# mlvlab/BLiM

Measured on AMD Instinct MI355X. Metric: candidate-pairs/sec (7B, 96+32 tok), higher is better.
Workload: dtype f16; 1 GPU; SYN v2t-VTG re-rank: Qwen2-7B dims (28 layers), seeded synthetic weights, 96 video + 32 text tokens per pair, top-16 text candidates per video query, 55 queries (880 pairs, 32560 packed tokens, 28160 label rows) per step per GPU; prefix_reuse=True, vtg_compensated=none, parallelism=query rows sharded over 1 GPU(s); RCCL all-gather of score rows at the end

## Files before the change

### blim_amd/csrc/attention.hip

```cpp
#include "attention.hpp"

#include <stdlib.h>

#include <type_traits>

#define HD 128
#define KT 32
#define QB 32

typedef __attribute__((ext_vector_type(4))) short s16x4;

template <int MAXC, bool SPLIT> struct attn_bound { static constexpr int value = MAXC <= (SPLIT ? 8 : 4) ? 512 : MAXC <= (SPLIT ? 16 : 8) ? 256 : 64; };
template <bool USE_TR, int MAXC, int DT, bool SPLIT = false, bool OUT_LO = SPLIT, bool PC = false>
__global__ __launch_bounds__((attn_bound<MAXC, SPLIT>::value)) void attn_kernel(const typename std::conditional<PC, AttnPcParams, AttnParams>::type p) {
    __shared__ __attribute__((aligned(16))) bf16_t k_lds[(SPLIT ? 2 : 1) * KT * HD];
    __shared__ __attribute__((aligned(16))) bf16_t v_lds[(SPLIT ? 2 : 1) * KT * HD];
    __shared__ uint32_t vis_lds[KT / 4];

    const int tid = threadIdx.x, nthreads = blockDim.x;
    const int lane = tid & 63;
    const int wave = tid >> 6;
    const int G = p.num_heads / p.num_kv_heads;
    const int ngrp = (int)gridDim.y / p.num_kv_heads;
    const int kh = blockIdx.y / ngrp, hg = blockIdx.y - kh * ngrp;
    const int hpg = (G + ngrp - 1) / ngrp;
    const int wave_head = hg * hpg + wave;
    const bool worker = wave < hpg && wave_head < G;
    const int head = kh * G + (worker ? wave_head : 0);
    const int blk = blockIdx.x;
    const int s = p.blk_seq[blk], q0 = p.blk_q0[blk];
    const int sstart = p.seq_start[s], slen = p.seq_len[s];
    int plen = p.pfx_len[s];
    const int pstart = plen > 0 ? p.pfx_start[s] : 0;
    const bf16_t* cbase = nullptr;
    if constexpr (PC) {
        const int slot = p.pfx_slot[s];
        if (slot >= 0 && slot < p.pc_n_slots) { cbase = p.pfx_cache + (int64_t)slot * p.pc_slot_stride; plen = min(plen, p.pc_max_len); }
    }

    const int qi = lane & 31, hf = lane >> 5;
    const int qtok = sstart + min(q0 + qi, slen - 1);
    const int qstart = p.own_start ? p.own_start[qtok] : 0;
    const int koff = p.num_heads * HD + kh * HD;
    const int voff = (p.num_heads + p.num_kv_heads) * HD + kh * HD;

    bf16x8 qf[8];
    {
        const bf16_t* qrow = p.qkv + (int64_t)qtok * p.ldq + head * HD + 8 * hf;
#pragma unroll
        for (int ks = 0; ks < 8; ++ks) qf[ks] = *(const bf16x8*)(qrow + 16 * ks);
    }
    bf16x8 qf_lo[SPLIT ? 8 : 1];
    if constexpr (SPLIT) {
        const bf16_t* qrow = p.qkv + (int64_t)qtok * p.ldq + p.v_lo_off + head * HD + 8 * hf;
#pragma unroll
        for (int ks = 0; ks < 8; ++ks) qf_lo[ks] = *(const bf16x8*)(qrow + 16 * ks);
    }

    __builtin_amdgcn_s_waitcnt(0x0F70);
    const int n_ptiles = (plen + KT - 1) / KT;
    const int own_keys = min(q0 + QB, slen);
    const int n_tiles = n_ptiles + (own_keys + KT - 1) / KT;

    f32x16 o[4];
#pragma unroll
    for (int i = 0; i < 4; ++i)
#pragma unroll
        for (int r = 0; r < 16; ++r) o[i][r] = 0.f;
    const float NEG = -1.0e30f;
    float m_run = NEG, l_run = 0.f;
    const float c_log2 = p.scale * 1.4426950408889634f;

    constexpr int NCHUNK = SPLIT ? 2048 : 1024;
    uint4 st[MAXC];
    uint8_t st_vis = 0;
#pragma unroll
    for (int i = 0; i < MAXC; ++i) st[i] = make_uint4(0, 0, 0, 0);

    auto tile_desc = [&](int t, int& base_tok, int& k0, int& seg_len, bool& causal) __attribute__((always_inline)) {
        if (t < n_ptiles) { base_tok = pstart; k0 = t * KT; seg_len = plen; causal = false; }
        else { base_tok = sstart; k0 = (t - n_ptiles) * KT; seg_len = slen; causal = true; }
    };
    auto load_tile = [&](int t) __attribute__((always_inline)) {
        int base_tok, k0, seg_len; bool causal;
        tile_desc(t, base_tok, k0, seg_len, causal);
        if constexpr (PC) {
            if (cbase != nullptr && t < n_ptiles) {
                const int ck = kh * HD, cv = p.num_kv_heads * HD + kh * HD;
#pragma unroll
                for (int i = 0; i < MAXC; ++i) {
                    const int idx = tid + i * nthreads;
                    if (idx < NCHUNK) {
                        const int isv = idx >> 9, row = (idx >> 4) & 31, ch = idx & 15;
                        const int kk = min(k0 + row, seg_len - 1);
                        st[i] = *(const uint4*)(cbase + (int64_t)kk * p.pc_ld + (isv == 0 ? ck : isv == 1 ? cv : isv == 2 ? cv + p.pc_lo_off : ck + p.pc_lo_off) + 8 * ch);
                    }
                }
                if (tid < KT) st_vis = (k0 + tid < seg_len) ? (uint8_t)1 : (uint8_t)0;
                return;
            }
        }
#pragma unroll
        for (int i = 0; i < MAXC; ++i) {
            const int idx = tid + i * nthreads;
            if (idx < NCHUNK) {
                const int isv = idx >> 9, row = (idx >> 4) & 31, ch = idx & 15;
                const int kk = min(k0 + row, seg_len - 1);
                st[i] = *(const uint4*)(p.qkv + (int64_t)(base_tok + kk) * p.ldq + (isv == 0 ? koff : isv == 1 ? voff : isv == 2 ? voff + p.v_lo_off : koff + p.v_lo_off) + 8 * ch);
            }
        }
        if (tid < KT) {
            const int kk = k0 + tid;
            st_vis = (kk < seg_len) ? p.key_visible[base_tok + kk] : (uint8_t)0;
        }
    };
    auto store_tile = [&](int t) __attribute__((always_inline)) {
        int base_tok, k0, seg_len; bool causal;
        tile_desc(t, base_tok, k0, seg_len, causal);
#pragma unroll
        for (int i = 0; i < MAXC; ++i) {
            const int idx = tid + i * nthreads;
            if (idx < NCHUNK) {
                const int isv = idx >> 9, row = (idx >> 4) & 31, ch = idx & 15;
                if (isv == 1 || isv == 2) *(uint4*)(v_lds + (isv - 1) * KT * HD + row * HD + 8 * (ch ^ ((row & 3) << 2))) = st[i];
                else *(uint4*)(k_lds + (isv >> 1) * KT * HD + row * HD + 8 * (ch ^ (row & 15))) = st[i];
            }
        }
        if (tid < KT) ((uint8_t*)vis_lds)[tid] = st_vis ? 1 : 0;
    };

    load_tile(0);
    for (int t = 0; t < n_tiles; ++t) {
#if defined(ATTN_ABLATE) && ATTN_ABLATE == 1
        if (t == 0) { __syncthreads(); store_tile(t); __syncthreads(); }
#else
        __syncthreads();
        store_tile(t);
        __syncthreads();
        if (t + 1 < n_tiles) load_tile(t + 1);
#endif
#if defined(ATTN_ABLATE) && ATTN_ABLATE == 2
        continue;
#endif
        if (!worker) continue;

        int base_tok, k0, seg_len; bool causal;
        tile_desc(t, base_tok, k0, seg_len, causal);

        f32x16 sacc;
#pragma unroll
        for (int r = 0; r < 16; ++r) sacc[r] = 0.f;
        {
            const int key = lane & 31;
#pragma unroll
            for (int ks = 0; ks < 8; ++ks) {
                const bf16x8 kf = *(const bf16x8*)(k_lds + key * HD + 8 * ((2 * ks + hf) ^ (key & 15)));
                sacc = mfma32<DT>(kf, qf[ks], sacc);
                if constexpr (SPLIT) {
                    sacc = mfma32<DT>(kf, qf_lo[ks], sacc);
                    const bf16x8 kl = *(const bf16x8*)(k_lds + KT * HD + key * HD + 8 * ((2 * ks + hf) ^ (key & 15)));
                    sacc = mfma32<DT>(kl, qf[ks], sacc);
                }
            }
        }
        float pv[16];
        const bool vis_all = (vis_lds[0] & vis_lds[1] & vis_lds[2] & vis_lds[3] & vis_lds[4] & vis_lds[5] & vis_lds[6] & vis_lds[7]) == 0x01010101u;
        if (!vis_all || (causal && (k0 + KT - 1 > q0 || p.own_start != nullptr))) {
#pragma unroll
            for (int g = 0; g < 4; ++g) {
                const uint32_t vb = vis_lds[2 * g + hf];
#pragma unroll
                for (int j = 0; j < 4; ++j) {
                    const int r = 4 * g + j;
                    const int kk = k0 + 8 * g + 4 * hf + j;
                    const bool ok = (((vb >> (8 * j)) & 0xFF) != 0) & (!causal | ((kk <= q0 + qi) & (kk >= qstart)));
                    sacc[r] = ok ? sacc[r] : NEG;
                }
            }
        }
        float tmax = NEG;
#pragma unroll
        for (int r = 0; r < 16; ++r) tmax = fmaxf(tmax, sacc[r]);
        tmax = xhalf_max(tmax);
        float m_new = m_run;
        const bool move = tmax * c_log2 > m_run * c_log2 + 8.0f;
        if (__builtin_amdgcn_ballot_w64(move) != 0) {
            m_new = move ? fmaxf(m_run, tmax) : m_run;
            const float alpha = __builtin_amdgcn_exp2f((m_run - m_new) * c_log2);
            l_run *= alpha;
#pragma unroll
            for (int i = 0; i < 4; ++i)
#pragma unroll
                for (int r = 0; r < 16; ++r) o[i][r] *= alpha;
        }
        const float mc = m_new > 0.5f * NEG ? m_new * c_log2 : 0.f;
        float rsum = 0.f;
#pragma unroll
        for (int r = 0; r < 16; ++r) {
            const float e = __builtin_amdgcn_exp2f(fmaf(sacc[r], c_log2, -mc));
            pv[r] = e;
            rsum += e;
        }
        l_run += xhalf_sum(rsum);
        m_run = m_new;

        bf16x8 pf[2], pf_lo[2];
#pragma unroll
        for (int s2 = 0; s2 < 2; ++s2) {
            uint32_t w[4], wl[4];
#pragma unroll
            for (int j = 0; j < 4; ++j) {
                const float a_ = pv[8 * s2 + 2 * j], b_ = pv[8 * s2 + 2 * j + 1];
                w[j] = pack2<DT>(a_, b_);
                if constexpr (SPLIT) wl[j] = pack2<DT>(a_ - from16<DT>(to16<DT>(a_)), b_ - from16<DT>(to16<DT>(b_)));
            }
            pf[s2] = __builtin_bit_cast(bf16x8, make_uint4(w[0], w[1], w[2], w[3]));
            if constexpr (SPLIT) pf_lo[s2] = __builtin_bit_cast(bf16x8, make_uint4(wl[0], wl[1], wl[2], wl[3]));
        }
#pragma unroll
        for (int vp = 0; vp < (SPLIT ? 2 : 1); ++vp) {
        const bf16_t* vt = v_lds + vp * KT * HD;
#pragma unroll
        for (int db = 0; db < 4; ++db) {
#pragma unroll
            for (int s2 = 0; s2 < 2; ++s2) {
                bf16x8 vf;
                if constexpr (USE_TR) {
                    const int i16 = lane & 15, g16 = (lane >> 4) & 1;
                    const int dcol = 32 * db + 16 * g16 + 4 * (i16 & 3);
                    const int ch = dcol >> 3, within = dcol & 7;
                    const int kr0 = 16 * s2 + 4 * hf + (i16 >> 2);
                    const int kr1 = kr0 + 8;
                    const s16x4 lo = __builtin_amdgcn_ds_read_tr16_b64_v4i16(
                        (__attribute__((address_space(3))) s16x4*)(vt + kr0 * HD + 8 * (ch ^ ((kr0 & 3) << 2)) + within));
                    const s16x4 hi = __builtin_amdgcn_ds_read_tr16_b64_v4i16(
                        (__attribute__((address_space(3))) s16x4*)(vt + kr1 * HD + 8 * (ch ^ ((kr1 & 3) << 2)) + within));
                    vf = (bf16x8){lo[0], lo[1], lo[2], lo[3], hi[0], hi[1], hi[2], hi[3]};
                } else {
                    const int d = 32 * db + (lane & 31);
#pragma unroll
                    for (int j = 0; j < 8; ++j) {
                        const int kr = 16 * s2 + 8 * (j >> 2) + 4 * hf + (j & 3);
                        vf[j] = (short)vt[kr * HD + 8 * ((d >> 3) ^ ((kr & 3) << 2)) + (d & 7)];
                    }
                }
                o[db] = mfma32<DT>(vf, pf[s2], o[db]);
                if constexpr (SPLIT) { if (vp == 0) o[db] = mfma32<DT>(vf, pf_lo[s2], o[db]); }
            }
        }
        }
    }

    if (!worker) return;
    if (p.out8 != nullptr) {
        const float inv = l_run > 0.f ? 1.0f / l_run : 0.f;
        float a = 0.f;
#pragma unroll
        for (int db = 0; db < 4; ++db)
#pragma unroll
            for (int r = 0; r < 16; ++r) { o[db][r] *= inv; a = fmaxf(a, fabsf(o[db][r])); }
        a = xhalf_max(a);
        int e = 0;
        if (a > 0.f) {
            int ex; const float mant = frexpf(a * (1.0f / FP8_MAX), &ex);
            e = (mant == 0.5f) ? ex - 1 : ex;
            if (ldexpf(a, -e) > FP8_MAX) e += 1;
            e = max(-127, min(127, e));
        }
        const float qs = ldexpf(1.0f, -e);
        if (q0 + qi < slen) {
            const int64_t tok = sstart + q0 + qi;
            uint8_t* orow = p.out8 + tok * p.ldo8 + head * HD;
#pragma unroll
            for (int db = 0; db < 4; ++db)
#pragma unroll
                for (int g = 0; g < 4; ++g)
                    *(uint32_t*)(orow + 32 * db + 8 * g + 4 * hf) = pack_fp8x4(o[db][4 * g] * qs, o[db][4 * g + 1] * qs, o[db][4 * g + 2] * qs, o[db][4 * g + 3] * qs);
            if (hf == 0) {
                const int rl = (int)(tok & 255);
                p.out_mx[(int64_t)head * p.mx_stride + (tok >> 8) * 256 + ((rl >> 7) * 16 + (rl & 15)) * 8 + ((rl >> 4) & 7)] = (uint8_t)(e + 127);
            }
        }
        return;
    }
    if (q0 + qi < slen) {
        const float inv = l_run > 0.f ? 1.0f / l_run : 0.f;
        bf16_t* orow = p.out + (int64_t)(sstart + q0 + qi) * p.ldo + head * HD;
        if (p.lse_out && hf == 0) p.lse_out[(int64_t)(sstart + q0 + qi) * p.num_heads + head] = l_run > 0.f ? m_run * p.scale + __logf(l_run) : 1.0e30f;
#pragma unroll
        for (int db = 0; db < 4; ++db)
#pragma unroll
            for (int g = 0; g < 4; ++g) {
                const int d = 32 * db + 8 * g + 4 * hf;
                const float x0 = o[db][4 * g] * inv, x1 = o[db][4 * g + 1] * inv, x2 = o[db][4 * g + 2] * inv, x3 = o[db][4 * g + 3] * inv;
                *(uint2*)(orow + d) = make_uint2(pack2<DT>(x0, x1), pack2<DT>(x2, x3));
                if constexpr (OUT_LO)
                    *(uint2*)(orow + p.out_lo_off + d) = make_uint2(pack2<DT>(x0 - from16<DT>(to16<DT>(x0)), x1 - from16<DT>(to16<DT>(x1))),
                                                                    pack2<DT>(x2 - from16<DT>(to16<DT>(x2)), x3 - from16<DT>(to16<DT>(x3))));
            }
    }
}

static bool stages_tile(int maxc, const dim3& block, bool split) {
    if (maxc * (int)block.x >= (split ? 2048 : 1024)) return true;
    blim_set_error("attention: %d threads x %d staging chunks do not cover a tile's %d", (int)block.x, maxc, split ? 2048 : 1024);
    return false;
}

static int launch_attention_pc(const AttnPcParams& p, int G, hipStream_t stream) {
    const dim3 grid(p.n_blocks, p.num_kv_heads), block(64 * G);
    static const int g_split = getenv("BLIM_ATTN_HEAD_GROUPS") ? atoi(getenv("BLIM_ATTN_HEAD_GROUPS")) : 2;
#define ATTN_PC(MC, SP, OL, GRID, BLOCK)                                                                                           \
    do {                                                                                                                       \
        if (!stages_tile(MC, BLOCK, SP)) return BLIM_ERR_ARG;                                                                  \
        if (p.dtype == DT_F16) hipLaunchKernelGGL((attn_kernel<true, MC, DT_F16, SP, OL, true>), GRID, BLOCK, 0, stream, p);      \
        else hipLaunchKernelGGL((attn_kernel<true, MC, DT_BF16, SP, OL, true>), GRID, BLOCK, 0, stream, p);                   \
    } while (0)
    if (p.v_lo_off != 0) {
        if (p.out_lo_off) { if (G >= 7) ATTN_PC(5, true, true, grid, block); else ATTN_PC(4, true, true, grid, dim3(512)); }
        else { if (G >= 7) ATTN_PC(5, true, false, grid, block); else ATTN_PC(4, true, false, grid, dim3(512)); }
    } else if (p.out_lo_off != 0) {
        if (G >= 7 && g_split > 1) ATTN_PC(4, false, true, dim3(p.n_blocks, p.num_kv_heads * 2), dim3(64 * ((G + 1) / 2)));
        else if (G >= 5 && g_split > 1) ATTN_PC(8, false, true, dim3(p.n_blocks, p.num_kv_heads * 2), dim3(64 * ((G + 1) / 2)));
        else if (G >= 4) ATTN_PC(4, false, true, grid, block);
        else if (G >= 2) ATTN_PC(8, false, true, grid, block);
        else ATTN_PC(16, false, true, grid, block);
    } else {
        if (G >= 7 && g_split > 1) ATTN_PC(4, false, false, dim3(p.n_blocks, p.num_kv_heads * 2), dim3(64 * ((G + 1) / 2)));
        else if (G >= 5 && g_split > 1) ATTN_PC(8, false, false, dim3(p.n_blocks, p.num_kv_heads * 2), dim3(64 * ((G + 1) / 2)));
        else if (G >= 4) ATTN_PC(4, false, false, grid, block);
        else if (G >= 2) ATTN_PC(8, false, false, grid, block);
        else ATTN_PC(16, false, false, grid, block);
    }
#undef ATTN_PC
    hipError_t e = hipGetLastError();
    if (e != hipSuccess) { blim_set_error("attention launch failed: %s", hipGetErrorString(e)); return BLIM_ERR_HIP; }
    return BLIM_OK;
}

int launch_attention_cached(const AttnPcParams& p, hipStream_t stream) {
    ARG_CHECK(p.qkv && p.out && p.key_visible && p.seq_start && p.seq_len && p.pfx_start && p.pfx_len && p.blk_seq && p.blk_q0);
    ARG_CHECK(p.n_blocks > 0 && p.num_kv_heads > 0 && p.num_heads % p.num_kv_heads == 0);
    ARG_CHECK(p.ldq % 8 == 0 && p.ldo % 4 == 0);
    ARG_CHECK(p.pfx_cache && p.pfx_slot && p.pc_n_slots > 0 && p.pc_max_len > 0 && p.pc_ld % 8 == 0 && p.pc_lo_off % 8 == 0 && p.pc_slot_stride % 8 == 0 && p.pc_lo_off >= 0);
    ARG_CHECK((p.dtype == DT_F16 || p.dtype == DT_BF16) && p.v_lo_off >= 0 && p.out_lo_off >= 0 && p.v_lo_off % 8 == 0 && p.out_lo_off % 4 == 0);
    if (p.out8 || p.lse_out) { blim_set_error("attention: the prefix-cache forms write a 16-bit output and no lse"); return BLIM_ERR_ARG; }
    if (p.v_lo_off != 0 && p.pc_lo_off == 0) { blim_set_error("attention: a compensated call needs a prefix cache that holds lo parts"); return BLIM_ERR_ARG; }
    const int G = p.num_heads / p.num_kv_heads;
    if (G > 8) { blim_set_error("attention: %d query heads per kv head > 8 unsupported", G); return BLIM_ERR_ARG; }
    return launch_attention_pc(p, G, stream);
}

int launch_attention(const AttnParams& p, int use_tr_read, hipStream_t stream) {
    ARG_CHECK(p.qkv && p.out && p.key_visible && p.seq_start && p.seq_len && p.pfx_start && p.pfx_len && p.blk_seq && p.blk_q0);
    ARG_CHECK(p.n_blocks > 0 && p.num_kv_heads > 0 && p.num_heads % p.num_kv_heads == 0);
    ARG_CHECK(p.ldq % 8 == 0 && p.ldo % 4 == 0);
    const int G = p.num_heads / p.num_kv_heads;
    if (G > 8) { blim_set_error("attention: %d query heads per kv head > 8 unsupported", G); return BLIM_ERR_ARG; }
    const dim3 grid(p.n_blocks, p.num_kv_heads), block(64 * G);
    if (p.v_lo_off != 0 || p.out_lo_off != 0)
        ARG_CHECK((p.dtype == DT_F16 || p.dtype == DT_BF16) && p.v_lo_off >= 0 && p.out_lo_off >= 0 && p.v_lo_off % 8 == 0 && p.out_lo_off % 4 == 0 && !p.out8);
    if (p.v_lo_off != 0) {
#define ATTN_SPLIT(MC, BLOCK)                                                                                                       \
        do {                                                                                                                      \
            if (!stages_tile(MC, BLOCK, true)) return BLIM_ERR_ARG;                                                               \
            if (p.out_lo_off) {                                                                                                   \
                if (p.dtype == DT_F16) hipLaunchKernelGGL((attn_kernel<true, MC, DT_F16, true>), grid, BLOCK, 0, stream, p);       \
                else hipLaunchKernelGGL((attn_kernel<true, MC, DT_BF16, true>), grid, BLOCK, 0, stream, p);                    \
            } else {                                                                                                              \
                if (p.dtype == DT_F16) hipLaunchKernelGGL((attn_kernel<true, MC, DT_F16, true, false>), grid, BLOCK, 0, stream, p); \
                else hipLaunchKernelGGL((attn_kernel<true, MC, DT_BF16, true, false>), grid, BLOCK, 0, stream, p);              \
            }                                                                                                                     \
        } while (0)
        if (G >= 7) ATTN_SPLIT(5, block);
        else ATTN_SPLIT(4, dim3(512));
#undef ATTN_SPLIT
        hipError_t e2 = hipGetLastError();
        if (e2 != hipSuccess) { blim_set_error("attention launch failed: %s", hipGetErrorString(e2)); return BLIM_ERR_HIP; }
        return BLIM_OK;
    }
    static const int g_split = getenv("BLIM_ATTN_HEAD_GROUPS") ? atoi(getenv("BLIM_ATTN_HEAD_GROUPS")) : 2;
    if (p.out_lo_off != 0) {
#define ATTN_LO(MC, GRID, BLOCK)                                                                                                   \
        do {                                                                                                                     \
            if (!stages_tile(MC, BLOCK, false)) return BLIM_ERR_ARG;                                                             \
            if (p.dtype == DT_F16) hipLaunchKernelGGL((attn_kernel<true, MC, DT_F16, false, true>), GRID, BLOCK, 0, stream, p);   \
            else hipLaunchKernelGGL((attn_kernel<true, MC, DT_BF16, false, true>), GRID, BLOCK, 0, stream, p);                \
        } while (0)
        if (G >= 7 && g_split > 1) ATTN_LO(4, dim3(p.n_blocks, p.num_kv_heads * 2), dim3(64 * ((G + 1) / 2)));
        else if (G >= 5 && g_split > 1) ATTN_LO(8, dim3(p.n_blocks, p.num_kv_heads * 2), dim3(64 * ((G + 1) / 2)));
        else if (G >= 4) ATTN_LO(4, grid, block);
        else if (G >= 2) ATTN_LO(8, grid, block);
        else ATTN_LO(16, grid, block);
#undef ATTN_LO
        hipError_t e3 = hipGetLastError();
        if (e3 != hipSuccess) { blim_set_error("attention launch failed: %s", hipGetErrorString(e3)); return BLIM_ERR_HIP; }
        return BLIM_OK;
    }
#define ATTN_LAUNCH(TR, MC)                                                                             \
    do {                                                                                            \
        if (!stages_tile(MC, block, false)) return BLIM_ERR_ARG;                                    \
        if (p.dtype == DT_F16) hipLaunchKernelGGL((attn_kernel<TR, MC, DT_F16>), grid, block, 0, stream, p); \
        else hipLaunchKernelGGL((attn_kernel<TR, MC, DT_BF16>), grid, block, 0, stream, p);                \
    } while (0)
    if (G >= 5 && g_split > 1 && use_tr_read && !p.out8) {
        const int hpg = (G + 1) / 2;
        const dim3 grid2(p.n_blocks, p.num_kv_heads * 2), block2(64 * hpg);
        if (!stages_tile(hpg >= 4 ? 4 : 8, block2, false)) return BLIM_ERR_ARG;
        if (hpg >= 4) {
            if (p.dtype == DT_F16) hipLaunchKernelGGL((attn_kernel<true, 4, DT_F16>), grid2, block2, 0, stream, p);
            else hipLaunchKernelGGL((attn_kernel<true, 4, DT_BF16>), grid2, block2, 0, stream, p);
        } else {
            if (p.dtype == DT_F16) hipLaunchKernelGGL((attn_kernel<true, 8, DT_F16>), grid2, block2, 0, stream, p);
            else hipLaunchKernelGGL((attn_kernel<true, 8, DT_BF16>), grid2, block2, 0, stream, p);
        }
    } else if (G >= 4) { if (use_tr_read) ATTN_LAUNCH(true, 4); else ATTN_LAUNCH(false, 4); }
    else if (G >= 2) { if (use_tr_read) ATTN_LAUNCH(true, 8); else ATTN_LAUNCH(false, 8); }
    else { if (use_tr_read) ATTN_LAUNCH(true, 16); else ATTN_LAUNCH(false, 16); }
#undef ATTN_LAUNCH
    hipError_t e = hipGetLastError();
    if (e != hipSuccess) { blim_set_error("attention launch failed: %s", hipGetErrorString(e)); return BLIM_ERR_HIP; }
    return BLIM_OK;
}
```

### blim_amd/csrc/attention.hpp

```cpp
#pragma once
#include "common.hpp"

struct AttnParams {
    int dtype;
    const bf16_t* qkv;
    int64_t ldq;
    int num_heads, num_kv_heads;
    const uint8_t* key_visible;
    const int32_t* seq_start;
    const int32_t* seq_len;
    const int32_t* pfx_start;
    const int32_t* pfx_len;
    const int32_t* blk_seq;
    const int32_t* blk_q0;
    const int32_t* own_start;
    int n_blocks;
    bf16_t* out;
    int64_t ldo;
    float scale;
    int64_t v_lo_off, out_lo_off;
    uint8_t* out8;
    int64_t ldo8;
    uint8_t* out_mx;
    int64_t mx_stride;
    float* lse_out;
};

int launch_attention(const AttnParams& p, int use_tr_read, hipStream_t stream);

struct AttnPcParams : AttnParams {
    const bf16_t* pfx_cache;
    const int32_t* pfx_slot;
    int64_t pc_slot_stride, pc_ld, pc_lo_off;
    int pc_n_slots, pc_max_len;
};
int launch_attention_cached(const AttnPcParams& p, hipStream_t stream);
```

### include/blim.h

```cpp
#ifndef BLIM_H_
#define BLIM_H_
#include <stdint.h>
#ifdef __cplusplus
extern "C" {
#endif

#define BLIM_ABI_VERSION 9
#define BLIM_ERR_ARG (-1)
#define BLIM_ERR_HIP (-2)
#define BLIM_ERR_STATE (-3)
#define BLIM_ERR_NOMEM (-4)

#define BLIM_DTYPE_F32 0
#define BLIM_DTYPE_BF16 1

#define BLIM_COMPUTE_BF16 0
#define BLIM_COMPUTE_F16 1
#define BLIM_COMPUTE_F8 2

typedef struct blim_engine blim_engine;

typedef struct blim_config {
    int32_t vocab_size, hidden_size, intermediate_size, num_layers, num_heads, num_kv_heads;
    int32_t mm_hidden_size;
    int32_t num_clips;
    int32_t max_positions;
    int32_t compute_dtype;
    float rms_eps, rope_theta;
} blim_config;

typedef struct blim_batch {
    int64_t n_tokens;
    int32_t n_seqs;
    int32_t n_blocks;
    const int32_t* positions;
    const uint8_t* key_visible;
    const int32_t* seq_start;
    const int32_t* seq_len;
    const int32_t* pfx_start;
    const int32_t* pfx_len;
    const int32_t* blk_seq;
    const int32_t* blk_q0;
    const int32_t* own_start;
} blim_batch;

int blim_abi_version(void);
const char* blim_last_error(void);

int blim_create(const blim_config* cfg, blim_engine** out);
void blim_destroy(blim_engine* e);

int blim_load_weight(blim_engine* e, const char* name, const void* data, int32_t dtype, int32_t on_device);
int blim_init_synthetic_weights(blim_engine* e, uint64_t seed);
int blim_weights_ready(const blim_engine* e);

int blim_hash_device(const void* p, int64_t bytes, uint64_t out[2], void* stream);
int blim_weights_fingerprint(blim_engine* e, uint64_t out[2], void* stream);

int blim_load_adapter(blim_engine* e, const char* weight_name, const float* A, const float* B, int32_t lora_r, float lora_alpha);
int blim_clear_adapters(blim_engine* e);
int blim_num_adapters(blim_engine* e);

int blim_reserve(blim_engine* e, int64_t max_tokens, int64_t max_rows);

int blim_project_video(blim_engine* e, const void* feats, int64_t n_rows, int32_t which, void* out, void* stream);
int blim_group_mean(blim_engine* e, const void* in, int64_t n_out, int32_t group, void* out, void* stream);

int blim_assemble(blim_engine* e, const int32_t* src_index, int64_t n_tokens, const void* feats, void* out_embeds, void* stream);

int blim_decode(blim_engine* e, const blim_batch* b, const void* embeds, const int32_t* out_rows, int64_t n_out,
                void* out_hidden_bf16, float* out_hidden_f32, void* stream);

int blim_vtg_logprobs(blim_engine* e, const void* hidden_bf16, const int32_t* labels, int64_t n_rows, float* logprob, void* stream);
int blim_segment_mean(blim_engine* e, const float* logprob, const int32_t* row_start, int32_t n_pairs, int32_t mode, float* score, void* stream);

int blim_lm_head(blim_engine* e, const void* hidden_bf16, int64_t n_rows, float* logits, void* stream);
int blim_ce_rows(blim_engine* e, const float* logits, int64_t ld, int32_t n_cols, const int32_t* labels, int64_t n_rows, float* logprob, void* stream);

int blim_visual_head(blim_engine* e, const void* hidden_bf16, int64_t n_rows, void* out_bf16, void* stream);
int blim_visual_head_f32(blim_engine* e, const float* hidden_f32, int64_t n_rows, float* out_f32, void* stream);
int blim_tvg_scores(blim_engine* e, const void* vh_bf16, const void* vocab_bf16, int32_t n_vocab, const int32_t* labels,
                    int32_t n_pairs, float* score, void* stream);
int blim_tvg_logits(blim_engine* e, const void* vh_bf16, const void* vocab_bf16, int32_t n_vocab, int32_t n_pairs, float* logits, void* stream);
int blim_set_video_vocab(blim_engine* e, const float* vocab_f32, int32_t n_vocab, void* stream);
int blim_tvg_logits_f32(blim_engine* e, const float* vh_f32, int32_t n_pairs, float* logits, void* stream);

int blim_score_vtg(blim_engine* e, const blim_batch* b, const void* embeds, const int32_t* rows, const int32_t* labels,
                   int64_t n_rows, const int32_t* row_start, int32_t n_pairs, float* score, void* stream);
int blim_score_tvg(blim_engine* e, const blim_batch* b, const void* embeds, const int32_t* rows, const void* vocab_bf16,
                   int32_t n_vocab, const int32_t* labels, int32_t n_pairs, float* score, void* stream);

typedef struct blim_pc_admit { int32_t seq, slot, start, len, row; } blim_pc_admit;
typedef struct blim_prefix_cache blim_prefix_cache;
int64_t blim_prefix_cache_bytes(const blim_engine* e, int32_t n_slots, int32_t max_len, int32_t compensated);
int blim_prefix_cache_create(blim_engine* e, int32_t n_slots, int32_t max_len, int32_t compensated, blim_prefix_cache** out);
void blim_prefix_cache_destroy(blim_prefix_cache* c);
int blim_prefix_cache_fill(blim_engine* e, blim_prefix_cache* c, const blim_batch* b, const void* embeds, const int32_t* slot_of_seq, void* stream);
int blim_prefix_cache_slot_len(const blim_prefix_cache* c, int32_t slot);
int blim_score_vtg_cached(blim_engine* e, blim_prefix_cache* c, const blim_batch* b, const int32_t* pfx_slot, const int32_t* slots_used, int32_t n_used,
                          const void* embeds, const int32_t* rows, const int32_t* labels, int64_t n_rows, const int32_t* row_start, int32_t n_pairs,
                          float* score, void* stream);
int blim_score_tvg_cached(blim_engine* e, blim_prefix_cache* c, const blim_batch* b, const int32_t* pfx_slot, const int32_t* slots_used, int32_t n_used,
                          const void* embeds, const int32_t* rows, const void* vocab_bf16, int32_t n_vocab, const int32_t* labels, int32_t n_pairs,
                          float* score, void* stream);
int blim_score_vtg_admit(blim_engine* e, blim_prefix_cache* c, const blim_batch* b, const int32_t* pfx_slot, const int32_t* slots_used, int32_t n_used,
                         const blim_pc_admit* admits, int32_t n_admit, const void* embeds, const int32_t* rows, const int32_t* labels, int64_t n_rows,
                         const int32_t* row_start, int32_t n_pairs, float* score, void* stream);
int blim_score_tvg_admit(blim_engine* e, blim_prefix_cache* c, const blim_batch* b, const int32_t* pfx_slot, const int32_t* slots_used, int32_t n_used,
                         const blim_pc_admit* admits, int32_t n_admit, const void* embeds, const int32_t* rows, const void* vocab_bf16, int32_t n_vocab,
                         const int32_t* labels, int32_t n_pairs, float* score, void* stream);

#define BLIM_PC_TICKET_MAGIC 0x544B4350u
#define BLIM_PC_TICKET_LAYERS 256
typedef struct blim_pc_move { int32_t slot; int32_t len; int64_t offset; } blim_pc_move;
typedef struct blim_pc_ticket {
    uint32_t magic;
    int32_t len;
    int32_t num_layers, kv_w, hid_w;
    int32_t precise, embeds, mlp, layers, lo6, mqz, n_bits;
    uint64_t epoch;
    uint8_t bits[BLIM_PC_TICKET_LAYERS];
} blim_pc_ticket;
int64_t blim_prefix_cache_record_bytes(const blim_prefix_cache* c, int32_t len);
int blim_prefix_cache_export(blim_engine* e, blim_prefix_cache* c, const blim_pc_move* moves, int32_t n, void* staging, int64_t staging_bytes,
                             blim_pc_ticket* tickets_out, void* stream);
int blim_prefix_cache_import(blim_engine* e, blim_prefix_cache* c, const blim_pc_move* moves, int32_t n, const void* staging, int64_t staging_bytes,
                             const blim_pc_ticket* tickets, void* stream);

int blim_forward(blim_engine* e, const void* embeds, const uint8_t* mask, int32_t B, int32_t L, float* logits, float* hidden, void* stream);

int blim_fill_bell_bf16(void* out, int64_t n, uint64_t seed, const char* name, float std, float mean, void* stream);
int blim_fill_bell_f32(float* out, int64_t n, uint64_t seed, const char* name, float std, float mean, int32_t round_bf16, void* stream);
int blim_gemm_f16(const void* A, int64_t lda, const void* W, int32_t M, int32_t N, int32_t K, void* C, int64_t ldc, void* stream);
int blim_gemm_bf16(const void* A, int64_t lda, const void* W, int32_t M, int32_t N, int32_t K, void* C, int64_t ldc, void* stream);
int64_t blim_f6_tiles_bytes(int64_t n_rows, int32_t K);
int blim_gemm_f16_lo6(const void* A_hilo, const void* W, int32_t M, int32_t N, int32_t K, void* a6, void* w6, float* C, void* stream);
int blim_quant_rows(const void* in16, int64_t ld, int64_t n_rows, int32_t K, int32_t dtype16, void* out8, float* scale, void* stream);
int blim_gemm_f8(const void* A8, int64_t lda, const float* a_scale, const void* W8, const float* w_scale, int32_t M, int32_t N, int32_t K,
                 void* C, int64_t ldc, void* stream);
typedef struct blim_attention_args {
    int64_t struct_bytes;
    const blim_batch* batch;
    const void* qkv;
    int64_t ldq;
    int32_t num_heads, num_kv_heads;
    int32_t dtype16;
    int32_t use_tr_read;
    int64_t v_lo_off, out_lo_off;
    void* out;
    int64_t ldo;
    float scale;
    float* lse_out;
    void* out8;
    int64_t ldo8;
    void* out_mx;
    int64_t mx_stride;
    const void* pfx_cache;
    const int32_t* pfx_slot;
    int64_t pc_slot_stride, pc_ld, pc_lo_off;
    int32_t pc_n_slots, pc_max_len;
} blim_attention_args;
int blim_attention(const blim_attention_args* args, void* stream);

typedef struct blim_attention_bwd_args {
    int64_t struct_bytes;
    const void* qkv;
    int64_t ldq;
    const void* dout;
    int64_t ldo;
    const void* o16;
    int64_t ldo16;
    const float* lse;
    int32_t num_heads, num_kv_heads;
    int32_t dtype16;
    const uint8_t* key_visible;
    const int32_t* seq_start;
    const int32_t* seq_len;
    int32_t n_seqs, max_len;
    float scale;
    void* workspace;
    int64_t workspace_bytes;
    float* dqkv;
    int64_t n_tokens;
} blim_attention_bwd_args;
int64_t blim_attention_bwd_workspace_bytes(int64_t n_tokens, int32_t n_seqs, int32_t num_heads, int32_t max_len);
int blim_attention_bwd(const blim_attention_bwd_args* args, void* stream);
int blim_rope_bwd(void* out16, const float* dqkv, int64_t n_tokens, int32_t qkv_n, int32_t rope_cols, const int32_t* positions, const float* cos, const float* sin,
                  int32_t n_pos, int32_t dtype16, void* stream);


typedef struct blim_lora_down_args {
    int64_t struct_bytes;
    void* x16;
    int64_t ldx, T;
    int32_t K, n_adapters, r, dtype16;
    const float* A[3];
    float scale, drop_p;
    uint64_t seed;
    uint32_t site;
    int32_t reserved;
    void* workspace;
    int64_t workspace_bytes;
} blim_lora_down_args;
int64_t blim_lora_down_workspace_bytes(int32_t n_adapters, int32_t K);
int blim_lora_down(const blim_lora_down_args* args, void* stream);

#define BLIM_LORA_DB 1
#define BLIM_LORA_DU 2
#define BLIM_LORA_DA 4
typedef struct blim_lora_grads_args {
    int64_t struct_bytes;
    int32_t flags, dtype16;
    int64_t T;
    int32_t N, K, r, reserved;
    const void* dy16;
    int64_t ldy;
    const void* u16;
    int64_t ldu;
    const void* x16;
    int64_t ldx;
    const float* B;
    float scale, drop_p;
    uint64_t seed;
    uint32_t site;
    int32_t reserved2;
    float* dB;
    float* du;
    float* dA;
    void* workspace;
    int64_t workspace_bytes;
} blim_lora_grads_args;
int64_t blim_lora_grads_workspace_bytes(int32_t flags, int64_t T, int32_t N, int32_t K, int32_t r);
int blim_lora_grads(const blim_lora_grads_args* args, void* stream);

typedef struct blim_lora_dx_args {
    int64_t struct_bytes;
    float* dx;
    int64_t ldd, T;
    int32_t K, n_adapters, r, dtype16;
    const float* du[3];
    const float* A[3];
    float drop_p;
    uint32_t site;
    uint64_t seed;
    void* out16;
    int64_t ldo;
} blim_lora_dx_args;
int blim_lora_dx(const blim_lora_dx_args* args, void* stream);

typedef struct blim_rmsnorm_bwd_args {
    int64_t struct_bytes;
    float* dx;
    const float* dy;
    const float* x;
    const int32_t* rows;
    int64_t n_rows;
    int32_t H, accumulate;
    const float* w;
    float eps;
    int32_t dtype16;
    void* out16;
    int32_t n_adapters, r;
    const float* du[3];
    const float* A[3];
    float drop_p;
    uint32_t site;
    uint64_t seed;
} blim_rmsnorm_bwd_args;
int blim_rmsnorm_bwd(const blim_rmsnorm_bwd_args* args, void* stream);

int64_t blim_ce_workspace_bytes(int64_t n_rows);
int blim_ce_fwd_bwd(const float* logits, int64_t ldl, int32_t V, const int32_t* labels, int32_t label_div, int64_t n_rows, float coef, void* dl16, float* dl32,
                    int64_t ldd, float* loss, int32_t dtype16, void* workspace, int64_t workspace_bytes, void* stream);

int blim_gelu(int32_t backward, void* out16, int64_t ldo, const void* pre16, const float* dh, int64_t rows, int32_t H, int32_t dtype16, void* stream);

int blim_adamw_raw(float* p, const float* g, float* exp_avg, float* exp_avg_sq, int64_t n, float lr, float beta1, float beta2, float eps, float weight_decay,
                   float inv_scale, int32_t step, void* stream);
int64_t blim_grad_stats_workspace_bytes(int64_t n);
int blim_grad_stats_raw(const float* g, int64_t n, float inv_scale, float* stats, void* workspace, int64_t workspace_bytes, void* stream);

typedef struct blim_rmsnorm_args {
    int64_t struct_bytes;
    const float* x;
    int64_t ldx;
    const int32_t* rows;
    int64_t n_rows, n_src;
    int32_t H, dtype16;
    const float* w;
    float eps;
    int32_t saturate;
    void* out16;
    int64_t ldo;
    void* out_lo;
    float* out_f32;
    void* out6;
} blim_rmsnorm_args;
int blim_rmsnorm(const blim_rmsnorm_args* args, void* stream);
int blim_rmsnorm_f8(const float* x, int64_t ldx, int64_t n_rows, int32_t H, const float* w, float eps, void* out8, float* scale, void* stream);
int blim_lse_combine(const float* part, int32_t n_tiles, const float* label_logit, const int32_t* labels, int64_t n_rows, float* logprob, void* stream);
int blim_tvg_criterion(const float* logits, int64_t ld, int32_t n_vocab, const int32_t* labels, int32_t n_pairs, int32_t clips, float* score, void* stream);
int blim_group_mean_rows(void* out, const void* in, int64_t n_out, int32_t group, int32_t H, int32_t dtype16, int32_t split, void* stream);
int blim_assemble_rows(void* out, const int32_t* src_index, int64_t n_tokens, int32_t H, const void* table, const void* feats, int32_t split, void* stream);

#define BLIM_EPI_BF16 0
#define BLIM_EPI_F32 1
#define BLIM_EPI_RESID 2
#define BLIM_EPI_QKV 3
#define BLIM_EPI_SWIGLU 4
#define BLIM_EPI_LSE 5
typedef struct blim_gemm_args {
    int64_t struct_bytes;
    int32_t epi;
    int32_t dtype;
    const void* A;
    int64_t lda;
    const void* W;
    int32_t M, N, K;
    int32_t act;
    void* C;
    int64_t ldc;
    const float* bias;
    const float* resid_in;
    float scale;
    int32_t w_wrap_k;
    int64_t lo_off;
    int32_t f16_saturate;
    int32_t rope_cols;
    const float* rope_rows;
    int64_t rope_stride;
    const int32_t* labels;
    float* lse_part;
    float* label_logit;
    const float* row_scale;
    const float* col_scale;
    const void* a_mx;
    void* out8;
    void* out_mx;
    int64_t mx_stride;
    void* A6;
    void* W6;
    int32_t K6;
    int32_t f6_build;
    void* out6;
    void* swiglu_act;
    int64_t swiglu_act_ld;
    void* swiglu_gu;
    int64_t swiglu_ld;
    int32_t tile;
    int32_t tile_lo6;
    int32_t tile_qkv;
} blim_gemm_args;
int blim_gemm(const blim_gemm_args* args, void* stream);
int64_t blim_gemm_narrow_launches(void);
int32_t blim_gemm_narrow_threshold(void);
int64_t blim_gemm_narrow_lo6_launches(void);
int32_t blim_gemm_narrow_lo6_threshold(void);
int64_t blim_gemm_narrow_qkv_launches(void);
int32_t blim_gemm_narrow_qkv_threshold(void);
int64_t blim_rope_rows_bytes(int32_t max_positions);
int blim_rope_rows(const int32_t* positions, int64_t n_tokens, float rope_theta, int32_t max_positions, void* workspace, float* out, int64_t stride, void* stream);

int blim_timing_enable(blim_engine* e, int32_t on);
int blim_timing_num_classes(void);
const char* blim_timing_class_name(int32_t cls);
int blim_timing_report(blim_engine* e, double* ms, int64_t* calls, double* flops);

int blim_debug_read(blim_engine* e, const char* which, void* dst, int64_t bytes, void* stream);

int blim_debug_gemm_stamps(void* device_buf);

int blim_set_option(blim_engine* e, const char* key, int32_t value);

typedef struct blim_vision blim_vision;
typedef struct blim_vision_config {
    int32_t image_size;
    int32_t patch_size;
    int32_t num_frames;
    int32_t hidden_size;
    int32_t num_heads;
    int32_t mlp_hidden;
    int32_t depth;
    int32_t tome_tokens;
    int32_t compute_dtype;
} blim_vision_config;
int blim_vision_create(const blim_vision_config* cfg, blim_vision** out);
void blim_vision_destroy(blim_vision* v);
int blim_vision_load_weight(blim_vision* v, const char* name, const void* data, int32_t dtype, int32_t on_device);
int blim_vision_init_synthetic_weights(blim_vision* v, uint64_t seed);
int blim_vision_set_pos_embed(blim_vision* v, const float* table_host);
int blim_vision_ready(const blim_vision* v);
int blim_vision_encode(blim_vision* v, const void* frames, int32_t n_clips, float* out_feat, float* out_tome, void* stream);
int blim_vit_attention(const void* qkv, int32_t n_clips, int32_t L, int32_t heads, int32_t dtype16, void* out, void* stream);
int blim_tome_merge(blim_vision* v, const float* x, int32_t b, int32_t p, int32_t c, int32_t heads, int32_t target, float* out, void* stream);

typedef struct blim_trainer blim_trainer;
typedef struct blim_train_config {
    int32_t lora_r;
    float lora_alpha;
    float lora_dropout;
} blim_train_config;
int64_t blim_train_flat_size(const blim_engine* e, int32_t lora_r);
int blim_train_param_offset(const blim_engine* e, int32_t lora_r, const char* name, int64_t* offset, int64_t* rows, int64_t* cols);
int blim_train_create(blim_engine* e, const blim_train_config* cfg, float* params, float* grads, blim_trainer** out);
void blim_train_destroy(blim_trainer* t);
int blim_train_sync_params(blim_trainer* t, void* stream);
int blim_train_merge(blim_trainer* t, void* stream);
typedef struct blim_train_batch {
    const blim_batch* batch;
    const int32_t* src_index;
    const void* feats;
    int64_t n_feat_rows;
    int32_t tok_per_clip;
    int32_t max_seq_len;
    const int32_t* rows;
    const int32_t* labels;
    int64_t n_rows;
    const int32_t* tvg_rows;
    const int32_t* tvg_labels;
    int64_t n_tvg_rows;
    const void* vocab;
    int32_t n_vocab;
    float grad_scale;
    uint64_t dropout_seed;
} blim_train_batch;
int blim_train_step(blim_trainer* t, const blim_train_batch* b, float* loss_sums, void* stream);
int blim_train_grad_stats(blim_trainer* t, float inv_scale, float* stats, void* stream);
int blim_train_adamw(blim_trainer* t, float* exp_avg, float* exp_avg_sq, float lr, float beta1, float beta2, float eps, float weight_decay, float inv_scale,
                     int32_t step, void* stream);
int blim_train_debug_read(blim_trainer* t, const char* which, void* dst, int64_t bytes, void* stream);

#ifdef __cplusplus
}
#endif
#endif
```

Baseline: 2625 pairs/s.

## Issue first KV tile load before Q load and widen attention output stores

The first K/V tile's global loads now start before the query fragments are loaded and before the waitcnt, so both sets of memory latency overlap. The epilogue also gains a 16-byte store path that uses permlane32 swaps to gather each lane's output into full uint4 writes when alignment allows, replacing narrower scattered stores. Debug timestamp instrumentation and ablation switches are added too, gated on a null pointer by default. The cost is extra registers held live during the prologue, plus the cross-lane swap work in the epilogue.

```diff
diff --git a/blim_amd/csrc/attention.hip b/blim_amd/csrc/attention.hip
--- a/blim_amd/csrc/attention.hip
+++ b/blim_amd/csrc/attention.hip
@@ -43,33 +43,16 @@
     const int qstart = p.own_start ? p.own_start[qtok] : 0;
     const int koff = p.num_heads * HD + kh * HD;
     const int voff = (p.num_heads + p.num_kv_heads) * HD + kh * HD;
-
-    bf16x8 qf[8];
-    {
-        const bf16_t* qrow = p.qkv + (int64_t)qtok * p.ldq + head * HD + 8 * hf;
-#pragma unroll
-        for (int ks = 0; ks < 8; ++ks) qf[ks] = *(const bf16x8*)(qrow + 16 * ks);
-    }
-    bf16x8 qf_lo[SPLIT ? 8 : 1];
-    if constexpr (SPLIT) {
-        const bf16_t* qrow = p.qkv + (int64_t)qtok * p.ldq + p.v_lo_off + head * HD + 8 * hf;
-#pragma unroll
-        for (int ks = 0; ks < 8; ++ks) qf_lo[ks] = *(const bf16x8*)(qrow + 16 * ks);
-    }
-
-    __builtin_amdgcn_s_waitcnt(0x0F70);
+    unsigned long long ts[6] = {0, 0, 0, 0, 0, 0};
+    const bool stamping = p.debug_stamps != nullptr && __builtin_amdgcn_readfirstlane(wave) == 0;
+    auto stamp = [&](int k) __attribute__((always_inline)) {
+        if (stamping) ts[k] = __builtin_amdgcn_s_memrealtime();
+    };
+    stamp(0);
+
     const int n_ptiles = (plen + KT - 1) / KT;
     const int own_keys = min(q0 + QB, slen);
     const int n_tiles = n_ptiles + (own_keys + KT - 1) / KT;
-
-    f32x16 o[4];
-#pragma unroll
-    for (int i = 0; i < 4; ++i)
-#pragma unroll
-        for (int r = 0; r < 16; ++r) o[i][r] = 0.f;
-    const float NEG = -1.0e30f;
-    float m_run = NEG, l_run = 0.f;
-    const float c_log2 = p.scale * 1.4426950408889634f;
 
     constexpr int NCHUNK = SPLIT ? 2048 : 1024;
     uint4 st[MAXC];
@@ -114,6 +97,36 @@
             st_vis = (kk < seg_len) ? p.key_visible[base_tok + kk] : (uint8_t)0;
         }
     };
+
+#if !(defined(ATTN_ABLATE) && (ATTN_ABLATE == 4 || ATTN_ABLATE == 5))
+    load_tile(0);
+#endif
+
+    bf16x8 qf[8];
+    {
+        const bf16_t* qrow = p.qkv + (int64_t)qtok * p.ldq + head * HD + 8 * hf;
+#pragma unroll
+        for (int ks = 0; ks < 8; ++ks) qf[ks] = *(const bf16x8*)(qrow + 16 * ks);
+    }
+    bf16x8 qf_lo[SPLIT ? 8 : 1];
+    if constexpr (SPLIT) {
+        const bf16_t* qrow = p.qkv + (int64_t)qtok * p.ldq + p.v_lo_off + head * HD + 8 * hf;
+#pragma unroll
+        for (int ks = 0; ks < 8; ++ks) qf_lo[ks] = *(const bf16x8*)(qrow + 16 * ks);
+    }
+
+    __builtin_amdgcn_s_waitcnt(0x0F70);
+    stamp(1);
+
+    f32x16 o[4];
+#pragma unroll
+    for (int i = 0; i < 4; ++i)
+#pragma unroll
+        for (int r = 0; r < 16; ++r) o[i][r] = 0.f;
+    const float NEG = -1.0e30f;
+    float m_run = NEG, l_run = 0.f;
+    const float c_log2 = p.scale * 1.4426950408889634f;
+
     auto store_tile = [&](int t) __attribute__((always_inline)) {
         int base_tok, k0, seg_len; bool causal;
         tile_desc(t, base_tok, k0, seg_len, causal);
@@ -129,7 +142,9 @@
         if (tid < KT) ((uint8_t*)vis_lds)[tid] = st_vis ? 1 : 0;
     };
 
+#if defined(ATTN_ABLATE) && (ATTN_ABLATE == 4 || ATTN_ABLATE == 5)
     load_tile(0);
+#endif
     for (int t = 0; t < n_tiles; ++t) {
 #if defined(ATTN_ABLATE) && ATTN_ABLATE == 1
         if (t == 0) { __syncthreads(); store_tile(t); __syncthreads(); }
@@ -137,6 +152,7 @@
         __syncthreads();
         store_tile(t);
         __syncthreads();
+        if (stamping && ts[2] == 0) stamp(2);
         if (t + 1 < n_tiles) load_tile(t + 1);
 #endif
 #if defined(ATTN_ABLATE) && ATTN_ABLATE == 2
@@ -251,6 +267,7 @@
         }
     }
 
+    stamp(3);
     if (!worker) return;
     if (p.out8 != nullptr) {
         const float inv = l_run > 0.f ? 1.0f / l_run : 0.f;
@@ -283,10 +300,40 @@
         }
         return;
     }
-    if (q0 + qi < slen) {
-        const float inv = l_run > 0.f ? 1.0f / l_run : 0.f;
-        bf16_t* orow = p.out + (int64_t)(sstart + q0 + qi) * p.ldo + head * HD;
-        if (p.lse_out && hf == 0) p.lse_out[(int64_t)(sstart + q0 + qi) * p.num_heads + head] = l_run > 0.f ? m_run * p.scale + __logf(l_run) : 1.0e30f;
+    const bool live = q0 + qi < slen;
+    const float inv = l_run > 0.f ? 1.0f / l_run : 0.f;
+    bf16_t* orow = p.out + (int64_t)(sstart + q0 + qi) * p.ldo + head * HD;
+    if (live && p.lse_out && hf == 0) p.lse_out[(int64_t)(sstart + q0 + qi) * p.num_heads + head] = l_run > 0.f ? m_run * p.scale + __logf(l_run) : 1.0e30f;
+    if (p.store16) {
+        uint4 w[8], wl[OUT_LO ? 8 : 1];
+#pragma unroll
+        for (int db = 0; db < 4; ++db)
+#pragma unroll
+            for (int g = 0; g < 4; g += 2) {
+                float x[8];
+#pragma unroll
+                for (int j = 0; j < 8; ++j) x[j] = o[db][4 * g + j] * inv;
+                const auto r0 = __builtin_amdgcn_permlane32_swap(pack2<DT>(x[0], x[1]), pack2<DT>(x[4], x[5]), false, false);
+                const auto r1 = __builtin_amdgcn_permlane32_swap(pack2<DT>(x[2], x[3]), pack2<DT>(x[6], x[7]), false, false);
+                w[2 * db + (g >> 1)] = make_uint4(r0[0], r1[0], r0[1], r1[1]);
+                if constexpr (OUT_LO) {
+                    float y[8];
+#pragma unroll
+                    for (int j = 0; j < 8; ++j) y[j] = x[j] - from16<DT>(to16<DT>(x[j]));
+                    const auto l0 = __builtin_amdgcn_permlane32_swap(pack2<DT>(y[0], y[1]), pack2<DT>(y[4], y[5]), false, false);
+                    const auto l1 = __builtin_amdgcn_permlane32_swap(pack2<DT>(y[2], y[3]), pack2<DT>(y[6], y[7]), false, false);
+                    wl[2 * db + (g >> 1)] = make_uint4(l0[0], l1[0], l0[1], l1[1]);
+                }
+            }
+        if (live) {
+#pragma unroll
+            for (int i = 0; i < 8; ++i) {
+                const int d = 16 * i + 8 * hf;
+                *(uint4*)(orow + d) = w[i];
+                if constexpr (OUT_LO) *(uint4*)(orow + p.out_lo_off + d) = wl[i];
+            }
+        }
+    } else if (live) {
 #pragma unroll
         for (int db = 0; db < 4; ++db)
 #pragma unroll
@@ -299,6 +346,33 @@
                                                                     pack2<DT>(x2 - from16<DT>(to16<DT>(x2)), x3 - from16<DT>(to16<DT>(x3))));
             }
     }
+    if (stamping) {
+        stamp(4);
+        __builtin_amdgcn_s_waitcnt(0x0F70);
+        stamp(5);
+        if (tid == 0) {
+            unsigned long long* dst = p.debug_stamps + ((size_t)blockIdx.y * gridDim.x + blockIdx.x) * 8;
+#pragma unroll
+            for (int k = 0; k < 6; ++k) dst[k] = ts[k];
+        }
+    }
+}
+
+static unsigned long long* g_attn_stamps = nullptr;
+extern "C" int blim_debug_attn_stamps(void* device_buf) {
+    g_attn_stamps = (unsigned long long*)device_buf;
+    return BLIM_OK;
+}
+
+template <class P> static P with_launch_fields(const P& in) {
+    P p = in;
+#if defined(ATTN_ABLATE) && (ATTN_ABLATE == 3 || ATTN_ABLATE == 5)
+    p.store16 = 0;
+#else
+    p.store16 = ((uintptr_t)p.out % 16 == 0 && p.ldo % 8 == 0 && p.out_lo_off % 8 == 0) ? 1 : 0;
+#endif
+    p.debug_stamps = g_attn_stamps;
+    return p;
 }
 
 static bool stages_tile(int maxc, const dim3& block, bool split) {
@@ -338,7 +412,8 @@
     return BLIM_OK;
 }
 
-int launch_attention_cached(const AttnPcParams& p, hipStream_t stream) {
+int launch_attention_cached(const AttnPcParams& p_in, hipStream_t stream) {
+    const AttnPcParams p = with_launch_fields(p_in);
     ARG_CHECK(p.qkv && p.out && p.key_visible && p.seq_start && p.seq_len && p.pfx_start && p.pfx_len && p.blk_seq && p.blk_q0);
     ARG_CHECK(p.n_blocks > 0 && p.num_kv_heads > 0 && p.num_heads % p.num_kv_heads == 0);
     ARG_CHECK(p.ldq % 8 == 0 && p.ldo % 4 == 0);
@@ -351,7 +426,8 @@
     return launch_attention_pc(p, G, stream);
 }
 
-int launch_attention(const AttnParams& p, int use_tr_read, hipStream_t stream) {
+int launch_attention(const AttnParams& p_in, int use_tr_read, hipStream_t stream) {
+    const AttnParams p = with_launch_fields(p_in);
     ARG_CHECK(p.qkv && p.out && p.key_visible && p.seq_start && p.seq_len && p.pfx_start && p.pfx_len && p.blk_seq && p.blk_q0);
     ARG_CHECK(p.n_blocks > 0 && p.num_kv_heads > 0 && p.num_heads % p.num_kv_heads == 0);
     ARG_CHECK(p.ldq % 8 == 0 && p.ldo % 4 == 0);
diff --git a/blim_amd/csrc/attention.hpp b/blim_amd/csrc/attention.hpp
--- a/blim_amd/csrc/attention.hpp
+++ b/blim_amd/csrc/attention.hpp
@@ -24,6 +24,8 @@
     uint8_t* out_mx;
     int64_t mx_stride;
     float* lse_out;
+    int store16;
+    unsigned long long* debug_stamps;
 };
 
 int launch_attention(const AttnParams& p, int use_tr_read, hipStream_t stream);
diff --git a/include/blim.h b/include/blim.h
--- a/include/blim.h
+++ b/include/blim.h
@@ -369,6 +369,7 @@
 int blim_debug_read(blim_engine* e, const char* which, void* dst, int64_t bytes, void* stream);
 
 int blim_debug_gemm_stamps(void* device_buf);
+int blim_debug_attn_stamps(void* device_buf);
 
 int blim_set_option(blim_engine* e, const char* key, int32_t value);
 
```

Result: no change. 2628 pairs/s, median of 2 (+0.1%).
